# AY-Liu/Image-Editing-Framework

Hardware: AMD Instinct MI355X
Metric: denoising steps/sec (SD1.5 512x512 P2P edit step, UNet batch 4) (higher is better)
Workload: dtype f16x3; 1 GPU; sd15 UNet (859.5M params) P2P AttentionRefine edit step, 2 prompts x CFG = batch 4, 64x64 latents (512x512 px), 50-step DDIM, guidance 7.5, cross 0.8 / self 0.4, per-step null-text unconditional embeddings (P2P_NTI, edit_real.py); one independent edit per GPU; precision mode f16x3: fp32 storage; every contraction on split operands: hi + lo fp16 halves of each fp32 element, Ah Bh + Al Bh + Ah Bl =

## Files before the change

image-editing-framework_amd/csrc/cross_p2p_x3.hip:

```cpp
#include "ief_common.h"
#include "ief_params.h"
#include "x3_common.h"

template <int D>
__global__ __launch_bounds__(256, (D > 80) ? 1 : 2) void attn_cross_p2p_x3_kernel(const IefAttnF32Params p, const int* __restrict__ edit_src,
                                                                                  const int* __restrict__ edit_slot,
                                                                                  const float* __restrict__ MT,
                                                                                  const float* __restrict__ coef) {
    constexpr int DG = (D + 15) / 16;
    constexpr int DT = (D + 31) / 32;
    constexpr int KLD = DG * 16 + 8;
    constexpr int VLD = 100;
    constexpr int MLD = 100;
    constexpr float SQ = 1.f, SK = 1.f, SV = 1.f, SP = 16384.f, SM = 256.f;
    const float SPE = p.p_scale > 0.f ? p.p_scale : SP;
    constexpr int RK = 2 * 96 * KLD, RV = 2 * DT * 32 * VLD, RM = 2 * 96 * MLD;
    constexpr int RSZ = RK > RV ? (RK > RM ? RK : RM) : (RV > RM ? RV : RM);
    __shared__ __attribute__((aligned(16))) half_t smem_c[RSZ];
    __shared__ float cf[2 * 96];
    half_t* Kh = smem_c;
    half_t* Kl = Kh + 96 * KLD;
    half_t* Vh = smem_c;
    half_t* Vl = Vh + DT * 32 * VLD;
    half_t* Mh = smem_c;
    half_t* Ml = Mh + 96 * MLD;
    const int tid = threadIdx.x, lane = tid & 63, wid = tid >> 6;
    const int li = lane & 31, lh = lane >> 5;
    const int nqb = gridDim.x;
    const int lid = xcd_remap(blockIdx.x + nqb * blockIdx.y, nqb * gridDim.y);
    const int bh = lid / nqb, qb = lid - bh * nqb, b = bh / p.heads, h = bh - b * p.heads;
    const int src = edit_src ? edit_src[b] : -1;
    const int qi = qb * 128 + wid * 32 + li;
    const int nt = (p.L + 31) / 32;
    const float sc2 = p.scale * 1.44269504088896341f / (SQ * SK);
    for (int c = tid; c < (int)(sizeof(smem_c) / 16); c += 256) ((f32x4*)smem_c)[c] = f32x4{0.f, 0.f, 0.f, 0.f};
    __syncthreads();

    constexpr int KCH = 32 * (D / 4);
    constexpr int NLD = (KCH + 255) / 256;
    auto probs = [&](int br, f32x16 (&P)[3]) {
        const float* Q = p.Q + (long long)br * p.sQb + (long long)h * D;
        const float* Kp = p.K + (long long)br * p.sKb + (long long)h * D;
        half8_t qh[DG], ql[DG];
#pragma unroll
        for (int g = 0; g < DG; ++g) {
#pragma unroll
            for (int c2 = 0; c2 < 2; ++c2) {
                const int d0 = g * 16 + 8 * lh + 4 * c2;
                f32x4 v = {0.f, 0.f, 0.f, 0.f};
                if (qi < p.N && d0 < D) v = *(const f32x4*)(Q + (long long)qi * p.ldq + d0);
                half4 hh, ll;
                split4(v, SQ, hh, ll);
#pragma unroll
                for (int j = 0; j < 4; ++j) { qh[g][4 * c2 + j] = hh[j]; ql[g][4 * c2 + j] = ll[j]; }
            }
        }
        f32x4 rk[3][NLD];
#pragma unroll
        for (int t = 0; t < 3; ++t)
#pragma unroll
            for (int i = 0; i < NLD; ++i) {
                const int c = tid + 256 * i;
                const int row = c / (D / 4), ch = c - row * (D / 4);
                rk[t][i] = (t < nt && c < KCH && t * 32 + row < p.L) ? *(const f32x4*)(Kp + (long long)(t * 32 + row) * p.ldk + ch * 4)
                                                                     : f32x4{0.f, 0.f, 0.f, 0.f};
            }
        __syncthreads();
#pragma unroll
        for (int t = 0; t < 3; ++t)
#pragma unroll
            for (int i = 0; i < NLD; ++i) {
                const int c = tid + 256 * i;
                if (t < nt && c < KCH) {
                    const int row = c / (D / 4), ch = c - row * (D / 4);
                    half4 hh, ll;
                    split4(rk[t][i], SK, hh, ll);
                    *(half4*)(Kh + (t * 32 + row) * KLD + ch * 4) = hh;
                    *(half4*)(Kl + (t * 32 + row) * KLD + ch * 4) = ll;
                }
            }
        if (DG * 16 > D) {
            constexpr int PADC = (DG * 16 - D) / 4;
            for (int c = tid; c < 96 * PADC; c += 256) {
                const int row = c / PADC, ch = c - row * PADC;
                *(half4*)(Kh + row * KLD + D + ch * 4) = half4{0, 0, 0, 0};
                *(half4*)(Kl + row * KLD + D + ch * 4) = half4{0, 0, 0, 0};
            }
        }
        __syncthreads();
        float mx = -INFINITY;
#pragma unroll
        for (int t = 0; t < 3; ++t) {
#pragma unroll
            for (int r = 0; r < 16; ++r) P[t][r] = -INFINITY;
            if (t < nt) {
                f32x16 sacc;
#pragma unroll
                for (int r = 0; r < 16; ++r) sacc[r] = 0.f;
#pragma unroll
                for (int g = 0; g < DG; ++g) {
                    const half8_t kh = *(const half8_t*)(Kh + (t * 32 + li) * KLD + g * 16 + 8 * lh);
                    const half8_t kl = *(const half8_t*)(Kl + (t * 32 + li) * KLD + g * 16 + 8 * lh);
                    sacc = __builtin_amdgcn_mfma_f32_32x32x16_f16(kl, qh[g], sacc, 0, 0, 0);
                    sacc = __builtin_amdgcn_mfma_f32_32x32x16_f16(kh, ql[g], sacc, 0, 0, 0);
                    sacc = __builtin_amdgcn_mfma_f32_32x32x16_f16(kh, qh[g], sacc, 0, 0, 0);
                }
                if ((t + 1) * 32 > p.L) {
#pragma unroll
                    for (int r = 0; r < 16; ++r) {
                        const int key = t * 32 + (r & 3) + 8 * (r >> 2) + 4 * lh;
                        P[t][r] = key < p.L ? sacc[r] * sc2 : -INFINITY;
                        mx = fmaxf(mx, P[t][r]);
                    }
                } else {
#pragma unroll
                    for (int r = 0; r < 16; ++r) { P[t][r] = sacc[r] * sc2; mx = fmaxf(mx, P[t][r]); }
                }
            }
        }
        mx = fmaxf(mx, __shfl_xor(mx, 32));
        float ls = 0.f;
#pragma unroll
        for (int t = 0; t < 3; ++t)
#pragma unroll
            for (int r = 0; r < 16; ++r) { P[t][r] = __builtin_amdgcn_exp2f(P[t][r] - mx); ls += P[t][r]; }
        ls += __shfl_xor(ls, 32);
        const float inv = 1.0f / ls;
#pragma unroll
        for (int t = 0; t < 3; ++t)
#pragma unroll
            for (int r = 0; r < 16; ++r) P[t][r] *= inv;
    };
    auto split_p = [&](const f32x16& P, int s, half8_t& ph, half8_t& pl, float sp) {
#pragma unroll
        for (int c2 = 0; c2 < 2; ++c2) {
            const f32x4 v = {P[8 * s + 4 * c2], P[8 * s + 4 * c2 + 1], P[8 * s + 4 * c2 + 2], P[8 * s + 4 * c2 + 3]};
            half4 hh, ll;
            split4(v, sp, hh, ll);
#pragma unroll
            for (int j = 0; j < 4; ++j) { ph[4 * c2 + j] = hh[j]; pl[4 * c2 + j] = ll[j]; }
        }
    };

    f32x16 T[3];
    if (src >= 0) {
        const int slot = edit_slot[b];
        const float* mt = MT + (long long)slot * 96 * 96;
        f32x4 rm[9];
#pragma unroll
        for (int i = 0; i < 9; ++i) rm[i] = *(const f32x4*)(mt + (tid + 256 * i) * 4);
        if (tid < 192) cf[tid] = coef[(long long)slot * 192 + tid];
        f32x16 Ps[3];
        probs(src, Ps);
        __syncthreads();
#pragma unroll
        for (int i = 0; i < 9; ++i) {
            const int c = tid + 256 * i;
            const int w = c / 24, ch = c - w * 24;
            half4 hh, ll;
            split4(rm[i], SM, hh, ll);
            *(half4*)(Mh + w * MLD + ch * 4) = hh;
            *(half4*)(Ml + w * MLD + ch * 4) = ll;
        }
        __syncthreads();
        half8_t ph[6], pl[6];
#pragma unroll
        for (int s = 0; s < 6; ++s) split_p(Ps[s >> 1], s & 1, ph[s], pl[s], SP);
#pragma unroll
        for (int wt = 0; wt < 3; ++wt) {
#pragma unroll
            for (int r = 0; r < 16; ++r) T[wt][r] = 0.f;
#pragma unroll
            for (int s = 0; s < 6; ++s) {
                const half_t* mr = Mh + (wt * 32 + li) * MLD + 16 * s + 4 * lh;
                const half_t* mq = Ml + (wt * 32 + li) * MLD + 16 * s + 4 * lh;
                half8_t mh, ml;
                const half4 a0 = *(const half4*)mr, a1 = *(const half4*)(mr + 8);
                const half4 b0 = *(const half4*)mq, b1 = *(const half4*)(mq + 8);
#pragma unroll
                for (int j = 0; j < 4; ++j) { mh[j] = a0[j]; mh[4 + j] = a1[j]; ml[j] = b0[j]; ml[4 + j] = b1[j]; }
                T[wt] = __builtin_amdgcn_mfma_f32_32x32x16_f16(ml, ph[s], T[wt], 0, 0, 0);
                T[wt] = __builtin_amdgcn_mfma_f32_32x32x16_f16(mh, pl[s], T[wt], 0, 0, 0);
                T[wt] = __builtin_amdgcn_mfma_f32_32x32x16_f16(mh, ph[s], T[wt], 0, 0, 0);
            }
        }
    }
    const float* Vp = p.V + (long long)b * p.sVb + (long long)h * D;
    f32x4 rv[3][NLD];
#pragma unroll
    for (int t = 0; t < 3; ++t)
#pragma unroll
        for (int i = 0; i < NLD; ++i) {
            const int c = tid + 256 * i;
            const int row = c / (D / 4), ch = c - row * (D / 4);
            rv[t][i] = (t < nt && c < KCH && t * 32 + row < p.L) ? *(const f32x4*)(Vp + (long long)(t * 32 + row) * p.ldv + ch * 4)
                                                                 : f32x4{0.f, 0.f, 0.f, 0.f};
        }
    f32x16 P[3];
    probs(b, P);
    if (src >= 0) {
        const float invt = 1.0f / (SM * SP);
#pragma unroll
        for (int t = 0; t < 3; ++t)
#pragma unroll
            for (int r = 0; r < 16; ++r) {
                const int w = t * 32 + (r & 3) + 8 * (r >> 2) + 4 * lh;
                P[t][r] = cf[w] * (T[t][r] * invt) + cf[96 + w] * P[t][r];
            }
    }
    f32x16 o[DT];
#pragma unroll
    for (int tt = 0; tt < DT; ++tt)
#pragma unroll
        for (int r = 0; r < 16; ++r) o[tt][r] = 0.f;
    __syncthreads();
#pragma unroll
    for (int t = 0; t < 3; ++t)
#pragma unroll
        for (int i = 0; i < NLD; ++i) {
            const int c = tid + 256 * i;
            if (t < nt && c < KCH) {
                const int row = c / (D / 4), ch = c - row * (D / 4);
                half4 hh, ll;
                split4(rv[t][i], SV, hh, ll);
#pragma unroll
                for (int j = 0; j < 4; ++j) {
                    Vh[(ch * 4 + j) * VLD + t * 32 + row] = hh[j];
                    Vl[(ch * 4 + j) * VLD + t * 32 + row] = ll[j];
                }
            }
        }
    __syncthreads();
#pragma unroll
    for (int t = 0; t < 3; ++t) {
        if (t < nt) {
#pragma unroll
            for (int s = 0; s < 2; ++s) {
                half8_t ph, pl;
                split_p(P[t], s, ph, pl, SPE);
#pragma unroll
                for (int tt = 0; tt < DT; ++tt) {
                    const half_t* vr = Vh + (tt * 32 + li) * VLD + t * 32 + 16 * s + 4 * lh;
                    const half_t* vq = Vl + (tt * 32 + li) * VLD + t * 32 + 16 * s + 4 * lh;
                    half8_t vh, vl;
                    const half4 a0 = *(const half4*)vr, a1 = *(const half4*)(vr + 8);
                    const half4 b0 = *(const half4*)vq, b1 = *(const half4*)(vq + 8);
#pragma unroll
                    for (int j = 0; j < 4; ++j) { vh[j] = a0[j]; vh[4 + j] = a1[j]; vl[j] = b0[j]; vl[4 + j] = b1[j]; }
                    o[tt] = __builtin_amdgcn_mfma_f32_32x32x16_f16(vl, ph, o[tt], 0, 0, 0);
                    o[tt] = __builtin_amdgcn_mfma_f32_32x32x16_f16(vh, pl, o[tt], 0, 0, 0);
                    o[tt] = __builtin_amdgcn_mfma_f32_32x32x16_f16(vh, ph, o[tt], 0, 0, 0);
                }
            }
        }
    }
    const float inv = 1.0f / (SV * SPE);
    float* O = p.Out ? p.Out + (long long)b * p.sOb + (long long)h * D : nullptr;
    half_t* OP = p.OutP ? p.OutP + (long long)b * p.sOPb + (long long)h * D : nullptr;
    if (qi < p.N) {
#pragma unroll
        for (int tt = 0; tt < DT; ++tt)
#pragma unroll
            for (int g = 0; g < 4; ++g) {
                const int d = tt * 32 + 8 * g + 4 * lh;
                if (d < D) {
                    const f32x4 v = {o[tt][4 * g] * inv, o[tt][4 * g + 1] * inv, o[tt][4 * g + 2] * inv, o[tt][4 * g + 3] * inv};
                    if (O) *(f32x4*)(O + (long long)qi * p.ldo + d) = v;
                    if (OP) {
                        half4 hh, ll;
                        split4(v, 1.0f, hh, ll);
                        half_t* op = OP + (long long)qi * p.ldp + d;
                        *(half4*)op = hh;
                        *(half4*)(op + p.planeO) = ll;
                    }
                }
            }
    }
}

extern "C" int ief_attn_cross_p2p_f32(const IefAttnF32Params* pp, const int* edit_src, const int* edit_slot, const float* MT,
                                      const float* coef, void* stream) {
    if (!pp) return IEF_EINVAL;
    const IefAttnF32Params& p = *pp;
    if (!p.Q || !p.K || !p.V || (!p.Out && !p.OutP) || p.q_src || p.k_src || p.v_src) return IEF_EINVAL;
    if (p.OutP && ((p.ldp & 3) || (p.sOPb & 3) || (p.planeO & 3) || ((uintptr_t)p.OutP & 7))) return IEF_EALIGN;
    if (p.p_scale != 0.f && !(p.p_scale >= 1.f && p.p_scale <= 16384.f)) return IEF_EINVAL;
    if (edit_src && (!edit_slot || !MT || !coef)) return IEF_EINVAL;
    if (p.B <= 0 || p.heads <= 0 || p.N <= 0 || p.L <= 0 || p.L > 96) return IEF_ESHAPE;
    if ((p.ldq & 3) || (p.ldk & 3) || (p.ldv & 3) || (p.ldo & 3) || (p.sQb & 3) || (p.sKb & 3) || (p.sVb & 3) || (p.sOb & 3) ||
        (((uintptr_t)p.Q | (uintptr_t)p.K | (uintptr_t)p.V | (uintptr_t)(p.Out ? p.Out : p.Q) | (uintptr_t)(MT ? MT : p.Q)) & 15)) return IEF_EALIGN;
    hipStream_t st = (hipStream_t)stream;
    dim3 grid((p.N + 127) / 128, p.B * p.heads);
    switch (p.d) {
        case 40: hipLaunchKernelGGL(attn_cross_p2p_x3_kernel<40>, grid, dim3(256), 0, st, p, edit_src, edit_slot, MT, coef); break;
        case 64: hipLaunchKernelGGL(attn_cross_p2p_x3_kernel<64>, grid, dim3(256), 0, st, p, edit_src, edit_slot, MT, coef); break;
        case 80: hipLaunchKernelGGL(attn_cross_p2p_x3_kernel<80>, grid, dim3(256), 0, st, p, edit_src, edit_slot, MT, coef); break;
        case 160: hipLaunchKernelGGL(attn_cross_p2p_x3_kernel<160>, grid, dim3(256), 0, st, p, edit_src, edit_slot, MT, coef); break;
        default: return IEF_ESHAPE;
    }
    IEF_LAUNCH_CHECK();
    return IEF_OK;
}
```

Measured before the change: 74.56 steps/s.

## Make cross-attention P2P kernel persistent per head, keeping K/V/M resident in LDS

Restructures the cross-attention P2P kernel so each workgroup handles several query blocks of one (batch, head) pair. For head dims up to 80, the split K, V, source-K and mapper matrices are loaded into LDS once and reused across those blocks, and the next Q block is prefetched during the current block's compute. It also drops the LDS zero-fill, reorders batch/head assignment so edited batches are grouped and spread across XCDs, and forces launch bounds to 1 block per CU. The aim is to avoid repeating global K/V/M loads and splits per 128-query tile, at the cost of lower occupancy and fewer workgroups.

Result: no change. 74.64 steps/s (median of 6 runs) (+0.1%).

```diff
diff --git a/image-editing-framework_amd/csrc/cross_p2p_x3.hip b/image-editing-framework_amd/csrc/cross_p2p_x3.hip
--- a/image-editing-framework_amd/csrc/cross_p2p_x3.hip
+++ b/image-editing-framework_amd/csrc/cross_p2p_x3.hip
@@ -3,10 +3,10 @@
 #include "x3_common.h"
 
 template <int D>
-__global__ __launch_bounds__(256, (D > 80) ? 1 : 2) void attn_cross_p2p_x3_kernel(const IefAttnF32Params p, const int* __restrict__ edit_src,
-                                                                                  const int* __restrict__ edit_slot,
-                                                                                  const float* __restrict__ MT,
-                                                                                  const float* __restrict__ coef) {
+__global__ __launch_bounds__(256, 1) void attn_cross_p2p_x3_kernel(const IefAttnF32Params p, const int* __restrict__ edit_src,
+                                                                   const int* __restrict__ edit_slot, const float* __restrict__ MT,
+                                                                   const float* __restrict__ coef, const int wpp, const int bpw) {
+    constexpr bool RES = D <= 80;
     constexpr int DG = (D + 15) / 16;
     constexpr int DT = (D + 31) / 32;
     constexpr int KLD = DG * 16 + 8;
@@ -15,57 +15,59 @@
     constexpr float SQ = 1.f, SK = 1.f, SV = 1.f, SP = 16384.f, SM = 256.f;
     const float SPE = p.p_scale > 0.f ? p.p_scale : SP;
     constexpr int RK = 2 * 96 * KLD, RV = 2 * DT * 32 * VLD, RM = 2 * 96 * MLD;
-    constexpr int RSZ = RK > RV ? (RK > RM ? RK : RM) : (RV > RM ? RV : RM);
+    constexpr int OFF_V = RK, OFF_KS = RES ? RK + RV : 0, OFF_M = RES ? 2 * RK + RV : RK;
+    constexpr int RSZ = RES ? 2 * RK + RV + RM : RK + (RV > RM ? RV : RM);
+    static_assert(RSZ * 2 + 768 <= 160 * 1024 && (RK % 8) == 0 && (RV % 8) == 0, "LDS images");
     __shared__ __attribute__((aligned(16))) half_t smem_c[RSZ];
     __shared__ float cf[2 * 96];
     half_t* Kh = smem_c;
     half_t* Kl = Kh + 96 * KLD;
-    half_t* Vh = smem_c;
+    half_t* Vh = smem_c + OFF_V;
     half_t* Vl = Vh + DT * 32 * VLD;
-    half_t* Mh = smem_c;
+    half_t* Ksh = smem_c + OFF_KS;
+    half_t* Ksl = Ksh + 96 * KLD;
+    half_t* Mh = smem_c + OFF_M;
     half_t* Ml = Mh + 96 * MLD;
     const int tid = threadIdx.x, lane = tid & 63, wid = tid >> 6;
     const int li = lane & 31, lh = lane >> 5;
-    const int nqb = gridDim.x;
-    const int lid = xcd_remap(blockIdx.x + nqb * blockIdx.y, nqb * gridDim.y);
-    const int bh = lid / nqb, qb = lid - bh * nqb, b = bh / p.heads, h = bh - b * p.heads;
+    const int npair = p.B * p.heads;
+    const int lid = xcd_remap(blockIdx.x, gridDim.x);
+    const int slot = lid / wpp, wg = lid - slot * wpp;
+    const int ppx = npair >> 3;
+    const int rank = (npair & 7) == 0 ? (slot % ppx) * 8 + slot / ppx : slot;
+    const int rb = rank / p.heads, h = rank - rb * p.heads;
+    int b = rb;
+    if (edit_src) {
+        int ne = 0;
+        for (int i = 0; i < p.B; ++i) ne += edit_src[i] >= 0;
+        const bool want_e = rb < ne;
+        const int want = want_e ? rb : rb - ne;
+        int cnt = 0;
+        for (int i = 0; i < p.B; ++i)
+            if ((edit_src[i] >= 0) == want_e) {
+                if (cnt == want) b = i;
+                ++cnt;
+            }
+    }
     const int src = edit_src ? edit_src[b] : -1;
-    const int qi = qb * 128 + wid * 32 + li;
+    const int nblk = (p.N + 127) / 128;
+    const int qb0 = wg * bpw, qb1 = min(qb0 + bpw, nblk);
     const int nt = (p.L + 31) / 32;
     const float sc2 = p.scale * 1.44269504088896341f / (SQ * SK);
-    for (int c = tid; c < (int)(sizeof(smem_c) / 16); c += 256) ((f32x4*)smem_c)[c] = f32x4{0.f, 0.f, 0.f, 0.f};
-    __syncthreads();
 
     constexpr int KCH = 32 * (D / 4);
     constexpr int NLD = (KCH + 255) / 256;
-    auto probs = [&](int br, f32x16 (&P)[3]) {
-        const float* Q = p.Q + (long long)br * p.sQb + (long long)h * D;
-        const float* Kp = p.K + (long long)br * p.sKb + (long long)h * D;
-        half8_t qh[DG], ql[DG];
-#pragma unroll
-        for (int g = 0; g < DG; ++g) {
-#pragma unroll
-            for (int c2 = 0; c2 < 2; ++c2) {
-                const int d0 = g * 16 + 8 * lh + 4 * c2;
-                f32x4 v = {0.f, 0.f, 0.f, 0.f};
-                if (qi < p.N && d0 < D) v = *(const f32x4*)(Q + (long long)qi * p.ldq + d0);
-                half4 hh, ll;
-                split4(v, SQ, hh, ll);
-#pragma unroll
-                for (int j = 0; j < 4; ++j) { qh[g][4 * c2 + j] = hh[j]; ql[g][4 * c2 + j] = ll[j]; }
-            }
-        }
-        f32x4 rk[3][NLD];
+    auto load_kv = [&](const float* base, int ld, f32x4 (&r)[3][NLD]) {
 #pragma unroll
         for (int t = 0; t < 3; ++t)
 #pragma unroll
             for (int i = 0; i < NLD; ++i) {
-                const int c = tid + 256 * i;
+                const int c = min(tid + 256 * i, KCH - 1);
                 const int row = c / (D / 4), ch = c - row * (D / 4);
-                rk[t][i] = (t < nt && c < KCH && t * 32 + row < p.L) ? *(const f32x4*)(Kp + (long long)(t * 32 + row) * p.ldk + ch * 4)
-                                                                     : f32x4{0.f, 0.f, 0.f, 0.f};
-            }
-        __syncthreads();
+                r[t][i] = *(const f32x4*)(base + (long long)min(t * 32 + row, p.L - 1) * ld + ch * 4);
+            }
+    };
+    auto store_k = [&](const f32x4 (&r)[3][NLD], half_t* kh_, half_t* kl_) {
 #pragma unroll
         for (int t = 0; t < 3; ++t)
 #pragma unroll
@@ -74,20 +76,86 @@
                 if (t < nt && c < KCH) {
                     const int row = c / (D / 4), ch = c - row * (D / 4);
                     half4 hh, ll;
-                    split4(rk[t][i], SK, hh, ll);
-                    *(half4*)(Kh + (t * 32 + row) * KLD + ch * 4) = hh;
-                    *(half4*)(Kl + (t * 32 + row) * KLD + ch * 4) = ll;
+                    split4(t * 32 + row < p.L ? r[t][i] : f32x4{0.f, 0.f, 0.f, 0.f}, SK, hh, ll);
+                    *(half4*)(kh_ + (t * 32 + row) * KLD + ch * 4) = hh;
+                    *(half4*)(kl_ + (t * 32 + row) * KLD + ch * 4) = ll;
                 }
             }
         if (DG * 16 > D) {
             constexpr int PADC = (DG * 16 - D) / 4;
             for (int c = tid; c < 96 * PADC; c += 256) {
                 const int row = c / PADC, ch = c - row * PADC;
-                *(half4*)(Kh + row * KLD + D + ch * 4) = half4{0, 0, 0, 0};
-                *(half4*)(Kl + row * KLD + D + ch * 4) = half4{0, 0, 0, 0};
-            }
-        }
-        __syncthreads();
+                *(half4*)(kh_ + row * KLD + D + ch * 4) = half4{0, 0, 0, 0};
+                *(half4*)(kl_ + row * KLD + D + ch * 4) = half4{0, 0, 0, 0};
+            }
+        }
+    };
+    auto store_v = [&](const f32x4 (&r)[3][NLD]) {
+#pragma unroll
+        for (int t = 0; t < 3; ++t)
+#pragma unroll
+            for (int i = 0; i < NLD; ++i) {
+                const int c = tid + 256 * i;
+                if (t < nt && c < KCH) {
+                    const int row = c / (D / 4), ch = c - row * (D / 4);
+                    half4 hh, ll;
+                    split4(t * 32 + row < p.L ? r[t][i] : f32x4{0.f, 0.f, 0.f, 0.f}, SV, hh, ll);
+#pragma unroll
+                    for (int j = 0; j < 4; ++j) {
+                        Vh[(ch * 4 + j) * VLD + t * 32 + row] = hh[j];
+                        Vl[(ch * 4 + j) * VLD + t * 32 + row] = ll[j];
+                    }
+                }
+            }
+        if (DT * 32 > D) {
+            constexpr int PADR = DT * 32 - D;
+            for (int c = tid; c < PADR * (VLD / 4); c += 256) {
+                const int row = D + c / (VLD / 4), ch = c % (VLD / 4);
+                *(half4*)(Vh + row * VLD + ch * 4) = half4{0, 0, 0, 0};
+                *(half4*)(Vl + row * VLD + ch * 4) = half4{0, 0, 0, 0};
+            }
+        }
+    };
+    auto load_m = [&](const float* mt, f32x4 (&r)[9]) {
+#pragma unroll
+        for (int i = 0; i < 9; ++i) r[i] = *(const f32x4*)(mt + (tid + 256 * i) * 4);
+    };
+    auto store_m = [&](const f32x4 (&r)[9]) {
+#pragma unroll
+        for (int i = 0; i < 9; ++i) {
+            const int c = tid + 256 * i;
+            const int w = c / 24, ch = c - w * 24;
+            half4 hh, ll;
+            split4(r[i], SM, hh, ll);
+            *(half4*)(Mh + w * MLD + ch * 4) = hh;
+            *(half4*)(Ml + w * MLD + ch * 4) = ll;
+        }
+    };
+    auto load_q = [&](int br, int qb, f32x4 (&r)[DG][2]) {
+        const float* Q = p.Q + (long long)br * p.sQb + (long long)h * D;
+        const int qi = min(qb * 128 + wid * 32 + li, p.N - 1);
+#pragma unroll
+        for (int g = 0; g < DG; ++g)
+#pragma unroll
+            for (int c2 = 0; c2 < 2; ++c2) {
+                const int d0 = g * 16 + 8 * lh + 4 * c2;
+                f32x4 v = {0.f, 0.f, 0.f, 0.f};
+                if (d0 < D) v = *(const f32x4*)(Q + (long long)qi * p.ldq + d0);
+                r[g][c2] = v;
+            }
+    };
+    auto split_q = [&](const f32x4 (&r)[DG][2], half8_t (&qh)[DG], half8_t (&ql)[DG]) {
+#pragma unroll
+        for (int g = 0; g < DG; ++g)
+#pragma unroll
+            for (int c2 = 0; c2 < 2; ++c2) {
+                half4 hh, ll;
+                split4(r[g][c2], SQ, hh, ll);
+#pragma unroll
+                for (int j = 0; j < 4; ++j) { qh[g][4 * c2 + j] = hh[j]; ql[g][4 * c2 + j] = ll[j]; }
+            }
+    };
+    auto probs = [&](const half_t* kh_, const half_t* kl_, const half8_t (&qh)[DG], const half8_t (&ql)[DG], f32x16 (&P)[3]) {
         float mx = -INFINITY;
 #pragma unroll
         for (int t = 0; t < 3; ++t) {
@@ -99,8 +167,8 @@
                 for (int r = 0; r < 16; ++r) sacc[r] = 0.f;
 #pragma unroll
                 for (int g = 0; g < DG; ++g) {
-                    const half8_t kh = *(const half8_t*)(Kh + (t * 32 + li) * KLD + g * 16 + 8 * lh);
-                    const half8_t kl = *(const half8_t*)(Kl + (t * 32 + li) * KLD + g * 16 + 8 * lh);
+                    const half8_t kh = *(const half8_t*)(kh_ + (t * 32 + li) * KLD + g * 16 + 8 * lh);
+                    const half8_t kl = *(const half8_t*)(kl_ + (t * 32 + li) * KLD + g * 16 + 8 * lh);
                     sacc = __builtin_amdgcn_mfma_f32_32x32x16_f16(kl, qh[g], sacc, 0, 0, 0);
                     sacc = __builtin_amdgcn_mfma_f32_32x32x16_f16(kh, ql[g], sacc, 0, 0, 0);
                     sacc = __builtin_amdgcn_mfma_f32_32x32x16_f16(kh, qh[g], sacc, 0, 0, 0);
@@ -142,140 +210,178 @@
         }
     };
 
-    f32x16 T[3];
-    if (src >= 0) {
-        const int slot = edit_slot[b];
-        const float* mt = MT + (long long)slot * 96 * 96;
-        f32x4 rm[9];
-#pragma unroll
-        for (int i = 0; i < 9; ++i) rm[i] = *(const f32x4*)(mt + (tid + 256 * i) * 4);
-        if (tid < 192) cf[tid] = coef[(long long)slot * 192 + tid];
-        f32x16 Ps[3];
-        probs(src, Ps);
-        __syncthreads();
-#pragma unroll
-        for (int i = 0; i < 9; ++i) {
-            const int c = tid + 256 * i;
-            const int w = c / 24, ch = c - w * 24;
-            half4 hh, ll;
-            split4(rm[i], SM, hh, ll);
-            *(half4*)(Mh + w * MLD + ch * 4) = hh;
-            *(half4*)(Ml + w * MLD + ch * 4) = ll;
-        }
-        __syncthreads();
-        half8_t ph[6], pl[6];
-#pragma unroll
-        for (int s = 0; s < 6; ++s) split_p(Ps[s >> 1], s & 1, ph[s], pl[s], SP);
-#pragma unroll
-        for (int wt = 0; wt < 3; ++wt) {
-#pragma unroll
-            for (int r = 0; r < 16; ++r) T[wt][r] = 0.f;
-#pragma unroll
-            for (int s = 0; s < 6; ++s) {
-                const half_t* mr = Mh + (wt * 32 + li) * MLD + 16 * s + 4 * lh;
-                const half_t* mq = Ml + (wt * 32 + li) * MLD + 16 * s + 4 * lh;
-                half8_t mh, ml;
-                const half4 a0 = *(const half4*)mr, a1 = *(const half4*)(mr + 8);
-                const half4 b0 = *(const half4*)mq, b1 = *(const half4*)(mq + 8);
-#pragma unroll
-                for (int j = 0; j < 4; ++j) { mh[j] = a0[j]; mh[4 + j] = a1[j]; ml[j] = b0[j]; ml[4 + j] = b1[j]; }
-                T[wt] = __builtin_amdgcn_mfma_f32_32x32x16_f16(ml, ph[s], T[wt], 0, 0, 0);
-                T[wt] = __builtin_amdgcn_mfma_f32_32x32x16_f16(mh, pl[s], T[wt], 0, 0, 0);
-                T[wt] = __builtin_amdgcn_mfma_f32_32x32x16_f16(mh, ph[s], T[wt], 0, 0, 0);
-            }
-        }
-    }
+    const float* Kp = p.K + (long long)b * p.sKb + (long long)h * D;
     const float* Vp = p.V + (long long)b * p.sVb + (long long)h * D;
-    f32x4 rv[3][NLD];
-#pragma unroll
-    for (int t = 0; t < 3; ++t)
-#pragma unroll
-        for (int i = 0; i < NLD; ++i) {
-            const int c = tid + 256 * i;
-            const int row = c / (D / 4), ch = c - row * (D / 4);
-            rv[t][i] = (t < nt && c < KCH && t * 32 + row < p.L) ? *(const f32x4*)(Vp + (long long)(t * 32 + row) * p.ldv + ch * 4)
-                                                                 : f32x4{0.f, 0.f, 0.f, 0.f};
-        }
-    f32x16 P[3];
-    probs(b, P);
-    if (src >= 0) {
-        const float invt = 1.0f / (SM * SP);
-#pragma unroll
-        for (int t = 0; t < 3; ++t)
-#pragma unroll
-            for (int r = 0; r < 16; ++r) {
-                const int w = t * 32 + (r & 3) + 8 * (r >> 2) + 4 * lh;
-                P[t][r] = cf[w] * (T[t][r] * invt) + cf[96 + w] * P[t][r];
-            }
-    }
-    f32x16 o[DT];
-#pragma unroll
-    for (int tt = 0; tt < DT; ++tt)
-#pragma unroll
-        for (int r = 0; r < 16; ++r) o[tt][r] = 0.f;
-    __syncthreads();
-#pragma unroll
-    for (int t = 0; t < 3; ++t)
-#pragma unroll
-        for (int i = 0; i < NLD; ++i) {
-            const int c = tid + 256 * i;
-            if (t < nt && c < KCH) {
-                const int row = c / (D / 4), ch = c - row * (D / 4);
-                half4 hh, ll;
-                split4(rv[t][i], SV, hh, ll);
-#pragma unroll
-                for (int j = 0; j < 4; ++j) {
-                    Vh[(ch * 4 + j) * VLD + t * 32 + row] = hh[j];
-                    Vl[(ch * 4 + j) * VLD + t * 32 + row] = ll[j];
-                }
-            }
-        }
-    __syncthreads();
-#pragma unroll
-    for (int t = 0; t < 3; ++t) {
-        if (t < nt) {
-#pragma unroll
-            for (int s = 0; s < 2; ++s) {
-                half8_t ph, pl;
-                split_p(P[t], s, ph, pl, SPE);
-#pragma unroll
-                for (int tt = 0; tt < DT; ++tt) {
-                    const half_t* vr = Vh + (tt * 32 + li) * VLD + t * 32 + 16 * s + 4 * lh;
-                    const half_t* vq = Vl + (tt * 32 + li) * VLD + t * 32 + 16 * s + 4 * lh;
-                    half8_t vh, vl;
-                    const half4 a0 = *(const half4*)vr, a1 = *(const half4*)(vr + 8);
-                    const half4 b0 = *(const half4*)vq, b1 = *(const half4*)(vq + 8);
-#pragma unroll
-                    for (int j = 0; j < 4; ++j) { vh[j] = a0[j]; vh[4 + j] = a1[j]; vl[j] = b0[j]; vl[4 + j] = b1[j]; }
-                    o[tt] = __builtin_amdgcn_mfma_f32_32x32x16_f16(vl, ph, o[tt], 0, 0, 0);
-                    o[tt] = __builtin_amdgcn_mfma_f32_32x32x16_f16(vh, pl, o[tt], 0, 0, 0);
-                    o[tt] = __builtin_amdgcn_mfma_f32_32x32x16_f16(vh, ph, o[tt], 0, 0, 0);
-                }
-            }
-        }
-    }
-    const float inv = 1.0f / (SV * SPE);
+    const float* Ksp = p.K + (long long)(src >= 0 ? src : b) * p.sKb + (long long)h * D;
+    const float* mt = MT + (long long)(src >= 0 ? edit_slot[b] : 0) * 96 * 96;
     float* O = p.Out ? p.Out + (long long)b * p.sOb + (long long)h * D : nullptr;
     half_t* OP = p.OutP ? p.OutP + (long long)b * p.sOPb + (long long)h * D : nullptr;
-    if (qi < p.N) {
+
+    f32x4 rq[DG][2], rqs[DG][2];
+    if constexpr (RES) {
+        load_q(b, qb0, rq);
+        if (src >= 0) load_q(src, qb0, rqs);
+    }
+    if (src >= 0 && tid < 192) cf[tid] = coef[(long long)edit_slot[b] * 192 + tid];
+    if constexpr (RES) {
+        f32x4 rk[3][NLD], rv[3][NLD];
+        if (src >= 0) {
+            f32x4 rks[3][NLD], rm[9];
+            load_kv(Ksp, p.ldk, rks);
+            load_m(mt, rm);
+            load_kv(Kp, p.ldk, rk);
+            load_kv(Vp, p.ldv, rv);
+            store_k(rks, Ksh, Ksl);
+            store_m(rm);
+        } else {
+            load_kv(Kp, p.ldk, rk);
+            load_kv(Vp, p.ldv, rv);
+        }
+        store_k(rk, Kh, Kl);
+        store_v(rv);
+        __syncthreads();
+    }
+    half8_t qh[DG], ql[DG], qsh[DG], qsl[DG];
+    if constexpr (RES) {
+        split_q(rq, qh, ql);
+        if (src >= 0) split_q(rqs, qsh, qsl);
+    }
+
+    for (int qb = qb0; qb < qb1; ++qb) {
+        const bool more = RES && qb + 1 < qb1;
+        if (more) {
+            load_q(b, qb + 1, rq);
+            if (src >= 0) load_q(src, qb + 1, rqs);
+        }
+        [[maybe_unused]] f32x4 rk[3][NLD], rv[3][NLD];
+        f32x16 T[3];
+        if (src >= 0) {
+            if constexpr (!RES) {
+                f32x4 rks[3][NLD], rm[9];
+                load_q(src, qb, rqs);
+                load_kv(Ksp, p.ldk, rks);
+                load_m(mt, rm);
+                if (qb > qb0) __syncthreads();
+                split_q(rqs, qsh, qsl);
+                store_k(rks, Ksh, Ksl);
+                store_m(rm);
+                load_kv(Kp, p.ldk, rk);
+                load_kv(Vp, p.ldv, rv);
+                __syncthreads();
+            }
+            f32x16 Ps[3];
+            probs(Ksh, Ksl, qsh, qsl, Ps);
+            half8_t ph[6], pl[6];
+#pragma unroll
+            for (int s = 0; s < 6; ++s) split_p(Ps[s >> 1], s & 1, ph[s], pl[s], SP);
+#pragma unroll
+            for (int wt = 0; wt < 3; ++wt) {
+#pragma unroll
+                for (int r = 0; r < 16; ++r) T[wt][r] = 0.f;
+#pragma unroll
+                for (int s = 0; s < 6; ++s) {
+                    const half_t* mr = Mh + (wt * 32 + li) * MLD + 16 * s + 4 * lh;
+                    const half_t* mq = Ml + (wt * 32 + li) * MLD + 16 * s + 4 * lh;
+                    half8_t mh, ml;
+                    const half4 a0 = *(const half4*)mr, a1 = *(const half4*)(mr + 8);
+                    const half4 b0 = *(const half4*)mq, b1 = *(const half4*)(mq + 8);
+#pragma unroll
+                    for (int j = 0; j < 4; ++j) { mh[j] = a0[j]; mh[4 + j] = a1[j]; ml[j] = b0[j]; ml[4 + j] = b1[j]; }
+                    T[wt] = __builtin_amdgcn_mfma_f32_32x32x16_f16(ml, ph[s], T[wt], 0, 0, 0);
+                    T[wt] = __builtin_amdgcn_mfma_f32_32x32x16_f16(mh, pl[s], T[wt], 0, 0, 0);
+                    T[wt] = __builtin_amdgcn_mfma_f32_32x32x16_f16(mh, ph[s], T[wt], 0, 0, 0);
+                }
+            }
+        } else if constexpr (!RES) {
+            load_kv(Kp, p.ldk, rk);
+            load_kv(Vp, p.ldv, rv);
+        }
+        if constexpr (!RES) {
+            load_q(b, qb, rq);
+            __syncthreads();
+            store_k(rk, Kh, Kl);
+            store_v(rv);
+            split_q(rq, qh, ql);
+            __syncthreads();
+        }
+        f32x16 P[3];
+        probs(Kh, Kl, qh, ql, P);
+        if (src >= 0) {
+            const float invt = 1.0f / (SM * SP);
+#pragma unroll
+            for (int t = 0; t < 3; ++t)
+#pragma unroll
+                for (int r = 0; r < 16; ++r) {
+                    const int w = t * 32 + (r & 3) + 8 * (r >> 2) + 4 * lh;
+                    P[t][r] = cf[w] * (T[t][r] * invt) + cf[96 + w] * P[t][r];
+                }
+        }
+        f32x16 o[DT];
 #pragma unroll
         for (int tt = 0; tt < DT; ++tt)
 #pragma unroll
-            for (int g = 0; g < 4; ++g) {
-                const int d = tt * 32 + 8 * g + 4 * lh;
-                if (d < D) {
-                    const f32x4 v = {o[tt][4 * g] * inv, o[tt][4 * g + 1] * inv, o[tt][4 * g + 2] * inv, o[tt][4 * g + 3] * inv};
-                    if (O) *(f32x4*)(O + (long long)qi * p.ldo + d) = v;
-                    if (OP) {
-                        half4 hh, ll;
-                        split4(v, 1.0f, hh, ll);
-                        half_t* op = OP + (long long)qi * p.ldp + d;
-                        *(half4*)op = hh;
-                        *(half4*)(op + p.planeO) = ll;
+            for (int r = 0; r < 16; ++r) o[tt][r] = 0.f;
+#pragma unroll
+        for (int t = 0; t < 3; ++t) {
+            if (t < nt) {
+#pragma unroll
+                for (int s = 0; s < 2; ++s) {
+                    half8_t ph, pl;
+                    split_p(P[t], s, ph, pl, SPE);
+#pragma unroll
+                    for (int tt = 0; tt < DT; ++tt) {
+                        const half_t* vr = Vh + (tt * 32 + li) * VLD + t * 32 + 16 * s + 4 * lh;
+                        const half_t* vq = Vl + (tt * 32 + li) * VLD + t * 32 + 16 * s + 4 * lh;
+                        half8_t vh, vl;
+                        const half4 a0 = *(const half4*)vr, a1 = *(const half4*)(vr + 8);
+                        const half4 b0 = *(const half4*)vq, b1 = *(const half4*)(vq + 8);
+#pragma unroll
+                        for (int j = 0; j < 4; ++j) { vh[j] = a0[j]; vh[4 + j] = a1[j]; vl[j] = b0[j]; vl[4 + j] = b1[j]; }
+                        o[tt] = __builtin_amdgcn_mfma_f32_32x32x16_f16(vl, ph, o[tt], 0, 0, 0);
+                        o[tt] = __builtin_amdgcn_mfma_f32_32x32x16_f16(vh, pl, o[tt], 0, 0, 0);
+                        o[tt] = __builtin_amdgcn_mfma_f32_32x32x16_f16(vh, ph, o[tt], 0, 0, 0);
                     }
                 }
             }
-    }
+        }
+        if (more) {
+            split_q(rq, qh, ql);
+            if (src >= 0) split_q(rqs, qsh, qsl);
+        }
+        const float inv = 1.0f / (SV * SPE);
+        const int qi = qb * 128 + wid * 32 + li;
+        if (qi < p.N) {
+#pragma unroll
+            for (int tt = 0; tt < DT; ++tt)
+#pragma unroll
+                for (int g = 0; g < 4; ++g) {
+                    const int d = tt * 32 + 8 * g + 4 * lh;
+                    if (d < D) {
+                        const f32x4 v = {o[tt][4 * g] * inv, o[tt][4 * g + 1] * inv, o[tt][4 * g + 2] * inv, o[tt][4 * g + 3] * inv};
+                        if (O) *(f32x4*)(O + (long long)qi * p.ldo + d) = v;
+                        if (OP) {
+                            half4 hh, ll;
+                            split4(v, 1.0f, hh, ll);
+                            half_t* op = OP + (long long)qi * p.ldp + d;
+                            *(half4*)op = hh;
+                            *(half4*)(op + p.planeO) = ll;
+                        }
+                    }
+                }
+        }
+    }
+}
+
+static int cross_blocks_per_wg(int d, int nblk, int npair) {
+    if (d > 80) return 1;
+    static int ncu = 0;
+    if (ncu <= 0) {
+        int dev = 0, v = 0;
+        if (hipGetDevice(&dev) != hipSuccess || hipDeviceGetAttribute(&v, hipDeviceAttributeMultiprocessorCount, dev) != hipSuccess || v <= 0) v = 256;
+        ncu = v;
+    }
+    const int wpp = ncu / npair > 1 ? ncu / npair : 1;
+    return (nblk + wpp - 1) / wpp;
 }
 
 extern "C" int ief_attn_cross_p2p_f32(const IefAttnF32Params* pp, const int* edit_src, const int* edit_slot, const float* MT,
@@ -290,12 +396,15 @@
     if ((p.ldq & 3) || (p.ldk & 3) || (p.ldv & 3) || (p.ldo & 3) || (p.sQb & 3) || (p.sKb & 3) || (p.sVb & 3) || (p.sOb & 3) ||
         (((uintptr_t)p.Q | (uintptr_t)p.K | (uintptr_t)p.V | (uintptr_t)(p.Out ? p.Out : p.Q) | (uintptr_t)(MT ? MT : p.Q)) & 15)) return IEF_EALIGN;
     hipStream_t st = (hipStream_t)stream;
-    dim3 grid((p.N + 127) / 128, p.B * p.heads);
+    const int nblk = (p.N + 127) / 128, npair = p.B * p.heads;
+    const int bpw = cross_blocks_per_wg(p.d, nblk, npair), wpp = (nblk + bpw - 1) / bpw;
+    if ((long long)npair * wpp > 0x7fffffffLL) return IEF_ESHAPE;
+    dim3 grid(npair * wpp);
     switch (p.d) {
-        case 40: hipLaunchKernelGGL(attn_cross_p2p_x3_kernel<40>, grid, dim3(256), 0, st, p, edit_src, edit_slot, MT, coef); break;
-        case 64: hipLaunchKernelGGL(attn_cross_p2p_x3_kernel<64>, grid, dim3(256), 0, st, p, edit_src, edit_slot, MT, coef); break;
-        case 80: hipLaunchKernelGGL(attn_cross_p2p_x3_kernel<80>, grid, dim3(256), 0, st, p, edit_src, edit_slot, MT, coef); break;
-        case 160: hipLaunchKernelGGL(attn_cross_p2p_x3_kernel<160>, grid, dim3(256), 0, st, p, edit_src, edit_slot, MT, coef); break;
+        case 40: hipLaunchKernelGGL(attn_cross_p2p_x3_kernel<40>, grid, dim3(256), 0, st, p, edit_src, edit_slot, MT, coef, wpp, bpw); break;
+        case 64: hipLaunchKernelGGL(attn_cross_p2p_x3_kernel<64>, grid, dim3(256), 0, st, p, edit_src, edit_slot, MT, coef, wpp, bpw); break;
+        case 80: hipLaunchKernelGGL(attn_cross_p2p_x3_kernel<80>, grid, dim3(256), 0, st, p, edit_src, edit_slot, MT, coef, wpp, bpw); break;
+        case 160: hipLaunchKernelGGL(attn_cross_p2p_x3_kernel<160>, grid, dim3(256), 0, st, p, edit_src, edit_slot, MT, coef, wpp, bpw); break;
         default: return IEF_ESHAPE;
     }
     IEF_LAUNCH_CHECK();
```
